# zkonduit/ezkl

Measured on AMD Instinct MI355X. Metric: BN254 G1 MSM pts/s (2^20 points per GPU; NTT 2^22 elems/s in extra), higher is better.
Workload: dtype u32x8 (254-bit modular integer, Montgomery)

## Files before the change

ezkl_amd/csrc/msm.hip:

```cpp
#include "common.hpp"
#include <deque>
#include <thread>
#include <chrono>
#include "curve.hpp"
#include "curve29.hpp"
#include "host64.hpp"
#include <string.h>

namespace ezkl {

static constexpr uint32_t MSM_MAX_PART_BITS = 12;
static constexpr uint32_t MSM_SPAN_HEAVY = 16;
static constexpr uint32_t MSM_PART_STAGE = 13312;
static constexpr uint32_t MSM_BINSORT_STAGE = 15360;
static constexpr uint32_t MSM_HEAVY_CHUNK = 256;
static constexpr uint32_t MSM_DIGIT_E = 8;
static constexpr uint32_t MSM_LMIN = 8;
static constexpr uint32_t MSM_MAX_BIG = 64;
static constexpr uint32_t MSM_BIG_BLOCKS = 64;
static constexpr uint32_t MSM_BIG_ROWS = 8;

__device__ __forceinline__ uint32_t msm_part_of(uint32_t bucket, uint32_t NP) { return bucket ? 1u + (bucket & (NP - 1u)) : 0u; }
__device__ __forceinline__ uint32_t msm_lane_len(const uint32_t* offsets, uint32_t nb, uint32_t nlanes, uint32_t lmin) {
    const uint32_t l = (uint32_t)(((uint64_t)offsets[nb] + nlanes - 1) / nlanes);
// ... 92 lines not shown
    double best_cost = 0;
    for (uint32_t W = 10; W <= 127; W++) {
        WinPlan p{W, 254 / W, 254 % W};
        if (p.cmax() > 23) continue;
        const double cost = (double)n * W + 4.0 * (double)((size_t)1 << (p.cmax() - 1));
        if (!best.W || cost < best_cost) { best = p; best_cost = cost; }
    }
    return best;
}

__global__ __launch_bounds__(256) void msm_precompute_kernel(const g1a_t* prev, g1a_t* next, size_t n, uint32_t c) {
    size_t i = (size_t)blockIdx.x * blockDim.x + threadIdx.x;
    if (i >= n) return;
    g1a_t p = ld_g1a(prev + i);
    g1x_t a = g1x_from_affine(p);
    for (uint32_t k = 0; k < c; k++) a = g1x_double(a);
    st_g1a(next + i, g1x_to_affine(a));
}

__global__ __launch_bounds__(256) void msm_table_to_r261_kernel(g1a_t* tab, size_t count) {
    size_t i = (size_t)blockIdx.x * blockDim.x + threadIdx.x;
    if (i >= count) return;
    fe_t k;
#pragma unroll
    for (int q = 0; q < 8; q++) k.v[q] = Fq29C::R261_32[q];
    g1a_t p = ld_g1a(tab + i);
    if (g1a_is_id(p)) return;
    p.x = Fq::mul(p.x, k);
    p.y = Fq::mul(p.y, k);
    st_g1a(tab + i, p);
}

__device__ __forceinline__ bool gt_half_r(const fe_t& s) {
    uint32_t d[8], c = 0, br = 0;
#pragma unroll
    for (int i = 0; i < 8; i++) d[i] = addc32(s.v[i], s.v[i], c);
#pragma unroll
    for (int i = 0; i < 8; i++) (void)subb32(d[i], FrP::MOD[i], br);
    return c != 0 || br == 0;
}
__device__ __forceinline__ fe_t msm_canon(const fe_t* scalars, size_t i, uint32_t& neg) {
    fe_t s = Fr::from_mont(ld_fe(scalars + i));
    neg = 0;
    if (gt_half_r(s)) {
        uint32_t br = 0;
#pragma unroll
        for (int k = 0; k < 8; k++) s.v[k] = subb32(FrP::MOD[k], s.v[k], br);
        neg = 1;
    }
    return s;
}
__device__ __forceinline__ uint32_t msm_take_bits(fe_t& s, uint32_t c) {
    const uint32_t d = s.v[0] & ((1u << c) - 1u);
#pragma unroll
    for (int k = 0; k < 7; k++) s.v[k] = __builtin_amdgcn_alignbit(s.v[k + 1], s.v[k], c);
    s.v[7] >>= c;
    return d;
}
template <class F>
__device__ __forceinline__ void msm_foreach_digit(fe_t s, uint32_t neg, const WinPlan& wp, F&& f) {
    uint32_t carry = 0;
    for (uint32_t w = 0; w < wp.W; w++) {
        const uint32_t c = wp.width(w), half = 1u << (c - 1);
        uint32_t raw = msm_take_bits(s, c) + carry;
        if (raw > half) {
            carry = 1;
            if (raw != (1u << c)) f(w, (1u << c) - raw - 1u, neg ^ 1u);
        } else {
            carry = 0;
            if (raw) f(w, raw - 1u, neg);
        }
    }
}

__device__ __forceinline__ bool msm_digit_step(fe_t& s, uint32_t neg, uint32_t c, uint32_t& carry, uint32_t& bucket, uint32_t& sign) {
    const uint32_t half = 1u << (c - 1);
    const uint32_t raw = msm_take_bits(s, c) + carry;
    if (raw > half) {
        carry = 1;
        bucket = (1u << c) - raw - 1u;
        sign = neg ^ 1u;
        return raw != (1u << c);
    }
    carry = 0;
    bucket = raw - 1u;
    sign = neg;
    return raw != 0;
}

__device__ __forceinline__ uint32_t msm_block_scan(uint32_t v, uint32_t* wsum, uint32_t& total) {
    const uint32_t lane = threadIdx.x & 63u, wave = threadIdx.x >> 6, nw = blockDim.x >> 6;
    uint32_t x = v;
#pragma unroll
    for (uint32_t d = 1; d < 64; d <<= 1) {
        const uint32_t y = __shfl_up(x, d, 64);
        if (lane >= d) x += y;
    }
    if (lane == 63) wsum[wave] = x;
    __syncthreads();
    if (wave == 0) {
        uint32_t s = lane < nw ? wsum[lane] : 0u;
#pragma unroll
        for (uint32_t d = 1; d < 16; d <<= 1) {
            const uint32_t y = __shfl_up(s, d, 64);
            if (lane >= d) s += y;
        }
        if (lane < nw) wsum[lane] = s;
    }
    __syncthreads();
    total = wsum[nw - 1];
    const uint32_t r = x + (wave ? wsum[wave - 1] : 0u);
    __syncthreads();
    return r;
}

__global__ __launch_bounds__(256) void msm_hist_kernel(const fe_t* scalars, size_t n, size_t per_block, WinPlan wp,
                                                       uint32_t LB, uint32_t NP, uint32_t* wg_hist, uint32_t* wg_cnt,
                                                       const fe_t* const* scal_list, uint32_t* zero_base, uint32_t zero_words, size_t bstride) {
    BOFF(); BSH(wg_hist); BSH(wg_cnt);
    if (scal_list) scalars = scal_list[blockIdx.z];
    if (zero_base) {
        BSH(zero_base);
        for (uint32_t i = blockIdx.x * 256 + threadIdx.x; i < zero_words; i += gridDim.x * 256) zero_base[i] = 0;
    }
    __shared__ uint32_t lh[(1u << MSM_MAX_PART_BITS) + 1];
    const uint32_t NQ = NP + 1;
    for (uint32_t p = threadIdx.x; p < NQ; p += 256) lh[p] = 0;
    __syncthreads();
    size_t lo = (size_t)blockIdx.x * per_block, hi = lo + per_block < n ? lo + per_block : n;
    for (size_t i0 = lo + threadIdx.x; i0 < hi; i0 += 4 * 256) {
        fe_t s[4];
        uint32_t neg[4], carry[4] = {0, 0, 0, 0};
#pragma unroll
        for (int q = 0; q < 4; q++) {
            const size_t i = i0 + (size_t)q * 256;
            if (i < hi) s[q] = msm_canon(scalars, i, neg[q]);
            else { s[q] = Fr::zero(); neg[q] = 0; }
        }
        for (uint32_t w = 0; w < wp.W; w++) {
            const uint32_t c = wp.width(w);
#pragma unroll
            for (int q = 0; q < 4; q++) {
                uint32_t bucket, sign;
                if (msm_digit_step(s[q], neg[q], c, carry[q], bucket, sign)) atomicAdd(&lh[msm_part_of(bucket, NP)], 1u);
            }
        }
    }
    __syncthreads();
    for (uint32_t p = threadIdx.x; p < NQ; p += 256) {
        wg_hist[(size_t)blockIdx.x * NQ + p] = lh[p];
        wg_cnt[(size_t)blockIdx.x * NQ + p] = lh[p];
    }
}
__global__ __launch_bounds__(1024) void msm_hist_scan_kernel(uint32_t* wg_hist, uint32_t G, uint32_t NP, uint32_t* part_count, size_t bstride) {
    BOFF(); BSH(wg_hist); BSH(part_count);
    __shared__ uint32_t sums[32][33];
    const uint32_t c = threadIdx.x & 31, j = threadIdx.x >> 5;
    const uint32_t p = blockIdx.x * 32 + c;
    const uint32_t chunk = (G + 31) / 32, g0 = j * chunk, g1 = g0 + chunk < G ? g0 + chunk : G;
    uint32_t s = 0;
    if (p < NP)
        for (uint32_t g = g0; g < g1; g++) s += wg_hist[(size_t)g * NP + p];
    sums[j][c] = s;
    __syncthreads();
    if (j == 0) {
        uint32_t run = 0;
        for (uint32_t q = 0; q < 32; q++) {
            uint32_t v = sums[q][c];
            sums[q][c] = run;
            run += v;
        }
        if (p < NP) part_count[p] = run;
    }
    __syncthreads();
    if (p < NP) {
        uint32_t run = sums[j][c];
        for (uint32_t g = g0; g < g1; g++) {
            uint32_t v = wg_hist[(size_t)g * NP + p];
            wg_hist[(size_t)g * NP + p] = run;
            run += v;
        }
    }
}
__device__ __forceinline__ void msm_part_scan_body(const uint32_t* part_count, uint32_t NQ, uint32_t* part_base, uint32_t* big_flag,
                                                   uint32_t* big_list, uint32_t* big_count, uint32_t* sh) {
    const uint32_t t = threadIdx.x;
    constexpr uint32_t PER = 5;
    uint32_t v[PER], sum = 0;
#pragma unroll
    for (uint32_t q = 0; q < PER; q++) {
        const uint32_t i = PER * t + q;
        v[q] = i < NQ ? part_count[i] : 0;
        sum += v[q];
    }
    uint32_t total;
    uint32_t run = msm_block_scan(sum, sh, total) - sum;
#pragma unroll
    for (uint32_t q = 0; q < PER; q++) {
        const uint32_t i = PER * t + q;
        if (i < NQ) part_base[i] = run;
        run += v[q];
    }
    if (t == 1023) part_base[NQ] = total;
#pragma unroll
    for (uint32_t q = 0; q < PER; q++) {
        const uint32_t i = PER * t + q;
        if (i == 0 || i >= NQ) continue;
        uint32_t slot = 0;
        if (v[q] > MSM_BINSORT_STAGE) {
            slot = atomicAdd(big_count, 1u);
            if (slot < MSM_MAX_BIG) big_list[slot] = i - 1;
            slot = slot < MSM_MAX_BIG ? slot + 1 : 0;
        }
        big_flag[i - 1] = slot;
    }
}
__global__ __launch_bounds__(1024) void msm_part_scan_kernel(const uint32_t* part_count, uint32_t NQ, uint32_t* part_base, uint32_t* big_flag,
                                                             uint32_t* big_list, uint32_t* big_count, size_t bstride) {
    BOFF(); BSH(part_count); BSH(part_base); BSH(big_flag); BSH(big_list); BSH(big_count);
    __shared__ uint32_t sh[1024];
    msm_part_scan_body(part_count, NQ, part_base, big_flag, big_list, big_count, sh);
}
__global__ __launch_bounds__(1024) void msm_partition_kernel(const fe_t* scalars, size_t n, size_t per_block, WinPlan wp,
                                                             uint32_t LB, uint32_t NP, size_t base_offset, size_t tab_stride,
                                                             const uint32_t* part_base, const uint32_t* wg_hist, const uint32_t* wg_cnt, uint2* entries,
                                                             uint32_t* vals, const fe_t* const* scal_list, size_t bstride) {
    BOFF(); BSH(part_base); BSH(wg_hist); BSH(wg_cnt); BSH(entries); BSH(vals);
    if (scal_list) scalars = scal_list[blockIdx.z];
    extern __shared__ uint32_t plds[];
    __shared__ uint32_t tsum[1024];
    const uint32_t NQ = NP + 1;
    uint32_t* start = plds;
    uint32_t* cursor = plds + (NQ + 1);
    uint32_t* gbase = plds + 2 * (NQ + 1);
    uint2* stage = reinterpret_cast<uint2*>(plds + 3 * (NQ + 1));
    const uint32_t t = threadIdx.x, T = blockDim.x;
    const uint32_t K = (NQ + T - 1) / T;
    uint32_t loc = 0;
    for (uint32_t q = 0; q < K; q++) {
        const uint32_t p = t * K + q;
        if (p < NQ) loc += wg_cnt[(size_t)blockIdx.x * NQ + p];
    }
    uint32_t total;
    uint32_t run = msm_block_scan(loc, tsum, total) - loc;
    for (uint32_t q = 0; q < K; q++) {
        const uint32_t p = t * K + q;
        if (p < NQ) {
            start[p] = run;
            cursor[p] = run;
            gbase[p] = part_base[p] + wg_hist[(size_t)blockIdx.x * NQ + p];
            run += wg_cnt[(size_t)blockIdx.x * NQ + p];
        }
    }
    __syncthreads();
    const size_t lo = (size_t)blockIdx.x * per_block, hi = lo + per_block < n ? lo + per_block : n;
    const size_t i = lo + t;
    if (i < hi) {
        uint32_t neg;
        fe_t s = msm_canon(scalars, i, neg);
        msm_foreach_digit(s, neg, wp, [&](uint32_t w, uint32_t bucket, uint32_t sign) {
            const uint32_t r = atomicAdd(&cursor[msm_part_of(bucket, NP)], 1u);
            stage[r] = make_uint2((uint32_t)(w * tab_stride + base_offset + i) | (sign << 31), bucket);
        });
    }
    __syncthreads();
    const uint32_t PB = 31 - __clz(NP);
    for (uint32_t idx = t; idx < total; idx += T) {
        const uint2 e = stage[idx];
        const uint32_t p = msm_part_of(e.y, NP);
        const uint32_t slot = gbase[p] + (idx - start[p]);
        if (p) entries[slot] = make_uint2(e.x, e.y >> PB);
        else vals[slot] = e.x;
    }
}
__device__ __forceinline__ uint32_t msm_wave_rank(uint32_t* cnt, uint32_t key) {
    const uint64_t active = __ballot(1);
    const uint32_t first = __builtin_amdgcn_readfirstlane(key);
    if (__ballot(key == first) == active) {
        const uint32_t rank = (uint32_t)__popcll(active & ((1ull << (threadIdx.x & 63u)) - 1ull));
        uint32_t base = 0;
        if (rank == 0) base = atomicAdd(&cnt[first], (uint32_t)__popcll(active));
        return (uint32_t)__builtin_amdgcn_readfirstlane(base) + rank;
    }
    return atomicAdd(&cnt[key], 1u);
}
__device__ __forceinline__ void msm_bins_scan(uint32_t* cnt, uint32_t* tsum, uint32_t nbins, uint32_t p, uint32_t beg, const uint32_t* part_base,
                                              bool emit, uint32_t* offsets, g1x29_t* buckets) {
    const uint32_t t = threadIdx.x;
    uint32_t loc[4], s = 0;
#pragma unroll
    for (int q = 0; q < 4; q++) {
        uint32_t j = t * 4 + q;
        loc[q] = j < nbins ? cnt[j] : 0;
        s += loc[q];
    }
    uint32_t total;
    uint32_t run = msm_block_scan(s, tsum, total) - s;
#pragma unroll
    for (int q = 0; q < 4; q++) {
        uint32_t j = t * 4 + q;
        if (j < nbins) {
            cnt[j] = run;
            if (emit) {
                const bool b0 = (p == 0 && j == 0);
                offsets[(size_t)p * nbins + j] = b0 ? part_base[0] : beg + run;
                if (b0 ? part_base[1] == part_base[0] : loc[q] == 0) st_f29(&buckets[(size_t)p * nbins + j].zz, Fq29::zero());
            }
        }
        run += loc[q];
    }
    __syncthreads();
}
__device__ __forceinline__ void msm_bigsort_count_body(const uint2* entries, const uint32_t* part_base, uint32_t LB, const uint32_t* big_list,
                                                       const uint32_t* big_count, uint32_t* bin_total, uint32_t* block_off, uint32_t* cnt, uint32_t bx,
                                                       uint32_t by, uint32_t rows);
__global__ __launch_bounds__(512) void msm_binsort_kernel(const uint2* entries, const uint32_t* part_base, uint32_t LB, uint32_t NP,
                                                          const uint32_t* big_flag, uint32_t* offsets, uint32_t* vals, g1x29_t* buckets,
                                                          const uint32_t* big_list, const uint32_t* big_count, uint32_t* bin_total, uint32_t* block_off,
                                                          size_t bstride) {
    BOFF(); BSH(entries); BSH(part_base); BSH(big_flag); BSH(offsets); BSH(vals); BSH(buckets);
    __shared__ uint32_t cnt[2048];
    __shared__ uint32_t tsum[512];
    extern __shared__ uint32_t stage[];
    if (blockIdx.x >= NP) {
        BSH(big_list); BSH(big_count); BSH(bin_total); BSH(block_off);
        const uint32_t w = blockIdx.x - NP;
        msm_bigsort_count_body(entries, part_base, LB, big_list, big_count, bin_total, block_off, cnt, w % MSM_BIG_BLOCKS, w / MSM_BIG_BLOCKS, MSM_BIG_ROWS);
        return;
// ... 97 lines not shown
                                                             uint32_t nb, uint32_t nlanes, g1x29_t* buckets, g1x29_t* head, g1x29_t* tail,
                                                             uint32_t* lane_first, uint32_t lmin, size_t bstride) {
    BOFF(); BSH(offsets); BSH(vals); BSH(buckets); BSH(head); BSH(tail); BSH(lane_first);
    const uint32_t t = blockIdx.x * blockDim.x + threadIdx.x;
    const uint32_t total = offsets[nb], L = msm_lane_len(offsets, nb, nlanes, lmin);
    const uint64_t k0w = (uint64_t)t * L;
    if (k0w >= total) return;
    const uint32_t k0 = (uint32_t)k0w;
    const uint32_t k1 = (uint64_t)k0 + L < total ? k0 + L : total;
    uint32_t lo = 0, hi = nb;
    while (hi - lo > 1) {
        uint32_t mid = (lo + hi) >> 1;
        if (offsets[mid] <= k0) lo = mid; else hi = mid;
    }
    uint32_t b = lo, bin_end = offsets[b + 1];
    uint32_t end_next = offsets[b + 2 <= nb ? b + 2 : nb];
    lane_first[t] = b;
    bool started_before = offsets[b] < k0;
    g1x29_t acc = g1x29_identity();
    MsmRec nxt = msm_fetch(tab, vals[k0]);
    uint32_t vn = k0 + 1 < k1 ? vals[k0 + 1] : 0u;
    for (uint32_t k = k0; k < k1; k++) {
        if (k == bin_end) {
            if (started_before) st_g1x29(head + t, acc); else st_g1x29(buckets + b, acc);
            acc.zz = Fq29::zero();
            started_before = false;
            b++;
            bin_end = end_next;
            if (bin_end == k) {
                uint32_t probes = 1;
                while (bin_end == k && probes < 4) { b++; bin_end = offsets[b + 1]; probes++; }
                if (bin_end == k) {
                    uint32_t lo2 = b + 1, hi2 = nb;
                    while (hi2 - lo2 > 1) {
                        uint32_t mid = (lo2 + hi2) >> 1;
                        if (offsets[mid] <= k) lo2 = mid; else hi2 = mid;
                    }
                    b = lo2;
                    bin_end = offsets[b + 1];
                }
            }
            end_next = offsets[b + 2 <= nb ? b + 2 : nb];
        }
        const MsmRec cur = nxt;
        nxt = msm_fetch(tab, vn);
        vn = k + 2 < k1 ? vals[k + 2] : 0u;
        acc = g1x29_add_mixed(acc, g1a29_unpack(cur.p), cur.neg);
    }
    if (k1 == bin_end) {
        if (started_before) st_g1x29(head + t, acc); else st_g1x29(buckets + b, acc);
    } else {
        if (started_before) st_g1x29(head + t, acc); else st_g1x29(tail + t, acc);
    }
}
EZ_D g1x29_t g1x29_shfl_down(const g1x29_t& p, uint32_t d) {
    g1x29_t r;
    const uint32_t* s = p.x.v;
    uint32_t* o = r.x.v;
#pragma unroll
    for (int k = 0; k < 36; k++) o[k] = __shfl_down(s[k], d);
    return r;
}
__global__ __launch_bounds__(256) void msm_fixup_boundary_tree_kernel(const uint32_t* offsets, uint32_t nb, uint32_t nlanes,
                                                                      const uint32_t* lane_first, const g1x29_t* head, const g1x29_t* tail, g1x29_t* buckets,
                                                                      uint32_t* heavy_list, uint32_t* heavy_count, uint32_t* chunk_list, uint32_t lmin,
                                                                      uint32_t span_heavy, size_t bstride) {
    BOFF(); BSH(offsets); BSH(lane_first); BSH(head); BSH(tail); BSH(buckets); BSH(heavy_list); BSH(heavy_count); BSH(chunk_list);
    const uint32_t t = blockIdx.x * blockDim.x + threadIdx.x + 1;
    const uint32_t lane = threadIdx.x & 63u;
    const uint32_t L = msm_lane_len(offsets, nb, nlanes, lmin);
    const uint64_t k0 = (uint64_t)t * L;
    bool cut = t < nlanes && k0 < offsets[nb];
    uint32_t b = 0, t1 = 0, t2 = 0;
    if (cut) {
        b = lane_first[t];
        const uint32_t beg = offsets[b], end = offsets[b + 1];
        cut = beg < k0;
        t1 = beg / L; t2 = (end - 1) / L;
    }
    if (cut && t2 - t1 > span_heavy) {
        if (t == t1 + 1 && t2 - t1 > MSM_HEAVY_CHUNK) heavy_list[atomicAdd(heavy_count, 1u)] = b;
        if ((t - t1 - 1) % MSM_HEAVY_CHUNK == 0) chunk_list[atomicAdd(heavy_count + 1, 1u)] = t;
        cut = false;
    }
    const uint32_t wave_last = t + (63u - lane);
    const uint32_t run = cut ? (t2 < wave_last ? t2 : wave_last) - t + 1u : 0u;
    uint32_t longest = run;
#pragma unroll
    for (uint32_t o = 32; o > 0; o >>= 1) {
        const uint32_t m = __shfl_xor(longest, o);
        longest = m > longest ? m : longest;
    }
    if (longest == 0) return;
    if (longest <= 2) {
        if (!cut || t != t1 + 1) return;
        g1x29_t acc = g1x29_add(ld_g1x29(tail + t1), ld_g1x29(head + t));
        for (uint32_t u = t + 1; u <= t2; u++) acc = g1x29_add(acc, ld_g1x29(head + u));
        st_g1x29(buckets + b, acc);
        return;
    }
    g1x29_t v = cut ? ld_g1x29(head + t) : g1x29_identity();
    uint32_t have = cut ? 1u : 0u;
#pragma unroll 1
    for (uint32_t d = 1; d < longest; d <<= 1) {
        const g1x29_t w = g1x29_shfl_down(v, d);
        const uint32_t hw = __shfl_down(have, d);
        if (have == d && run > d) {
            v = g1x29_add(v, w);
            have += hw;
        }
    }
    if (!cut || t != t1 + 1) return;
    g1x29_t acc = g1x29_add(ld_g1x29(tail + t1), v);
    for (uint32_t u = t + run; u <= t2; u++) acc = g1x29_add(acc, ld_g1x29(head + u));
    st_g1x29(buckets + b, acc);
}
__global__ __launch_bounds__(256) void msm_fixup_heavy1_kernel(const uint32_t* offsets, uint32_t nb, uint32_t nlanes, const uint32_t* lane_first, g1x29_t* head,
                                                               const g1x29_t* tail, g1x29_t* buckets, const uint32_t* chunk_list, const uint32_t* counts, uint32_t lmin,
                                                               uint32_t coop, size_t bstride) {
    BOFF(); BSH(offsets); BSH(lane_first); BSH(head); BSH(tail); BSH(buckets); BSH(chunk_list); BSH(counts);
    const uint32_t nchunks = counts[1], L = msm_lane_len(offsets, nb, nlanes, lmin);
    const uint32_t wave = threadIdx.x >> 6, lane = threadIdx.x & 63u;
    for (uint32_t ci = blockIdx.x * 4u + wave; ci < nchunks; ci += gridDim.x * 4u) {
        const uint32_t start = chunk_list[ci], b = lane_first[start];
        const uint32_t t2 = (offsets[b + 1] - 1) / L;
        const uint32_t stop = start + MSM_HEAVY_CHUNK - 1 < t2 ? start + MSM_HEAVY_CHUNK - 1 : t2;
        const uint32_t t1 = offsets[b] / L;
        const bool whole = t2 - t1 <= MSM_HEAVY_CHUNK;
        g1x29_t acc = (whole && lane == 63u) ? ld_g1x29(tail + t1) : g1x29_identity();
        for (uint32_t t = start + lane; t <= stop; t += 64) acc = g1x29_add(acc, ld_g1x29(head + t));
        acc = coop ? g1x29_group_sum_coop(acc, 64) : g1x29_group_sum(acc, 64);
        if (lane == 0) st_g1x29(whole ? buckets + b : head + start, acc);
    }
}
__global__ __launch_bounds__(256) void msm_fixup_heavy2_kernel(const uint32_t* offsets, uint32_t nb, uint32_t nlanes, const g1x29_t* head, const g1x29_t* tail,
                                                               const uint32_t* heavy_list, const uint32_t* counts, g1x29_t* buckets, uint32_t lmin, uint32_t coop, size_t bstride) {
    BOFF(); BSH(offsets); BSH(head); BSH(tail); BSH(heavy_list); BSH(counts); BSH(buckets);
    const uint32_t L = msm_lane_len(offsets, nb, nlanes, lmin);
    const uint32_t wave = threadIdx.x >> 6, lane = threadIdx.x & 63u;
    for (uint32_t h = blockIdx.x * 4u + wave; h < counts[0]; h += gridDim.x * 4u) {
        const uint32_t b = heavy_list[h];
        const uint32_t t1 = offsets[b] / L, t2 = (offsets[b + 1] - 1) / L;
        g1x29_t acc = lane == 63u ? ld_g1x29(tail + t1) : g1x29_identity();
        for (uint32_t t = t1 + 1 + lane * MSM_HEAVY_CHUNK; t <= t2; t += 64 * MSM_HEAVY_CHUNK) acc = g1x29_add(acc, ld_g1x29(head + t));
        acc = coop ? g1x29_group_sum_coop(acc, 64) : g1x29_group_sum(acc, 64);
        if (lane == 0) st_g1x29(buckets + b, acc);
    }
}

struct ReduceGeom {
    uint32_t wA, wB, wC;
    uint32_t wsA, wsB, wsC;
    uint32_t EA, GA, ET, GT;
};
__global__ __launch_bounds__(256, 2) void msm_reduce1_kernel(const g1x29_t* buckets, ReduceGeom g, g1x29_t* partA, g1x29_t* partT, size_t bstride) {
    BOFF(); BSH(buckets); BSH(partA); BSH(partT);
    const uint32_t idx = blockIdx.x * blockDim.x + threadIdx.x;
    g1x29_t acc = g1x29_identity();
    if (blockIdx.y == 0) {
        if (idx >= (g.GA << g.wA)) return;
        const uint32_t dA = idx & ((1u << g.wA) - 1u), grp = idx >> g.wA;
        for (uint32_t e = 0; e < g.EA; e++) acc = g1x29_add(acc, ld_g1x29(buckets + ((((size_t)grp * g.EA + e) << g.wA) | dA)));
        st_g1x29(partA + (size_t)dA * g.GA + grp, acc);
    } else {
        const uint32_t nT = 1u << (g.wB + g.wC);
        if (idx >= nT * g.GT) return;
        const uint32_t grp = idx % g.GT, t = idx / g.GT;
        for (uint32_t e = 0; e < g.ET; e++) acc = g1x29_add(acc, ld_g1x29(buckets + (((size_t)t << g.wA) | (e * g.GT + grp))));
        st_g1x29(partT + (size_t)t * g.GT + grp, acc);
    }
}
__global__ __launch_bounds__(64) void msm_reduce2_kernel(const g1x29_t* partA, const g1x29_t* partT, ReduceGeom g, g1x29_t* SA, g1x29_t* T, uint32_t lanesA,
                                                         uint32_t lanesT, uint32_t blocksA, uint32_t coop, size_t bstride) {
    BOFF(); BSH(partA); BSH(partT); BSH(SA); BSH(T);
    const bool isA = blockIdx.x < blocksA;
    const uint32_t lanes = isA ? lanesA : lanesT, per = 64 / lanes;
    const uint32_t o = (isA ? blockIdx.x : blockIdx.x - blocksA) * per + threadIdx.x / lanes, j = threadIdx.x % lanes;
    const uint32_t nout = isA ? (1u << g.wA) : (1u << (g.wB + g.wC)), G = isA ? g.GA : g.GT;
    g1x29_t acc = g1x29_identity();
    if (o < nout) {
        const g1x29_t* src = (isA ? partA : partT) + (size_t)o * G;
        for (uint32_t i = j; i < G; i += lanes) acc = g1x29_add(acc, ld_g1x29(src + i));
    }
    acc = (coop && lanes >= 4) ? g1x29_group_sum_coop(acc, lanes) : g1x29_group_sum(acc, lanes);
    if (j == 0 && o < nout) st_g1x29((isA ? SA : T) + o, acc);
}
__global__ __launch_bounds__(256) void msm_planes_kernel(const g1x29_t* SA, const g1x29_t* T, ReduceGeom g, g1x29_t* planes, g1x29_t* planes_host, uint32_t coop,
                                                         size_t bstride) {
    BOFF(); BSH(SA); BSH(T); BSH(planes);
    __shared__ uint4 sh[9 * 4];
    uint32_t id = blockIdx.x, field = 0, j = 0;
    if (id > 0) {
        id -= 1;
        if (id < g.wA) { field = 1; j = id; }
        else if (id < g.wA + g.wB) { field = 2; j = id - g.wA; }
        else { field = 3; j = id - g.wA - g.wB; }
    }
    const uint32_t nA = 1u << g.wA, nT = 1u << (g.wB + g.wC);
    g1x29_t acc = g1x29_identity();
    auto with_bit = [](uint32_t k, uint32_t bit) { return ((k >> bit) << (bit + 1)) | (1u << bit) | (k & ((1u << bit) - 1u)); };
    if (field == 0) {
        for (uint32_t d = threadIdx.x; d < nA; d += 256) acc = g1x29_add(acc, ld_g1x29(SA + d));
    } else if (field == 1) {
        for (uint32_t k = threadIdx.x; k < nA / 2; k += 256) acc = g1x29_add(acc, ld_g1x29(SA + with_bit(k, j)));
    } else {
        const uint32_t sh_bits = field == 2 ? j : g.wB + j;
        for (uint32_t k = threadIdx.x; k < nT / 2; k += 256) acc = g1x29_add(acc, ld_g1x29(T + with_bit(k, sh_bits)));
    }
    acc = (coop & 8u) ? g1x29_block256_sum_coop_full(acc, sh) : coop ? g1x29_block256_sum_coop(acc, sh) : g1x29_block256_sum(acc, sh);
    if (threadIdx.x == 0) {
        const uint32_t ws = field == 1 ? g.wsA : field == 2 ? g.wsB : g.wsC;
        const uint32_t slot = field == 0 ? 0u : 1u + ws + j;
        st_g1x29(planes + slot, acc);
        if (planes_host) st_g1x29(planes_host + (size_t)blockIdx.z * 32 + slot, acc);
    }
}

static int table_build(Ctx* c, hipStream_t st, const Bases* b, bool wait) {
    MsmTable t;
    t.n = b->n;
    t.wp = pick_plan(b->n);
    if ((size_t)t.wp.W * t.n >= ((size_t)1 << 31)) return EZKL_ERR_UNSUPPORTED;
    EZ_HIP(hipMalloc(&t.tab, (size_t)t.wp.W * t.n * sizeof(g1a_t)));
    EZ_HIP(hipMemcpyAsync(t.tab, b->pts, t.n * sizeof(g1a_t), hipMemcpyDeviceToDevice, st));
    for (uint32_t w = 1; w < t.wp.W; w++)
        hipLaunchKernelGGL(msm_precompute_kernel, dim3(cdiv(t.n, 256)), dim3(256), 0, st, t.tab + (size_t)(w - 1) * t.n,
                           t.tab + (size_t)w * t.n, t.n, t.wp.width(w - 1));
    hipLaunchKernelGGL(msm_table_to_r261_kernel, dim3(cdiv((size_t)t.wp.W * t.n, 256)), dim3(256), 0, st, t.tab, (size_t)t.wp.W * t.n);
    EZ_HIP(hipGetLastError());
    EZ_HIP(hipEventCreateWithFlags(&t.ready, hipEventDisableTiming));
    EZ_HIP(hipEventRecord(t.ready, st));
    if (wait) {
        EZ_HIP(hipStreamSynchronize(st));
        t.synced = true;
    }
    g_tables[b] = t;
    return EZKL_OK;
}
static int table_get(Ctx* c, hipStream_t st, const Bases* b, MsmTable** out) {
    auto it = g_tables.find(b);
    if (it == g_tables.end()) {
        int rc = table_build(c, st, b, true);
        if (rc) return rc;
        it = g_tables.find(b);
    }
    if (!it->second.synced) {
        EZ_HIP(hipEventSynchronize(it->second.ready));
        it->second.synced = true;
    }
    *out = &it->second;
    return EZKL_OK;
}
int msm_table_prepare(Ctx* c, const Bases* b) {
    if (g_tables.count(b)) return EZKL_OK;
    if (!g_table_stream) EZ_HIP(hipStreamCreateWithFlags(&g_table_stream, hipStreamNonBlocking));
    return table_build(c, g_table_stream, b, false);
}
void msm_table_drop(const Bases* b) {
    auto it = g_tables.find(b);
    if (it != g_tables.end()) {
        if (it->second.ready) { (void)hipEventSynchronize(it->second.ready); (void)hipEventDestroy(it->second.ready); }
        (void)hipFree(it->second.tab);
        g_tables.erase(it);
    }
}

static constexpr size_t MSM_MAX_GROUP = 16;
static int slot_prepare(MsmSlot& sl, size_t bytes, size_t msms = 1) {
    if (!sl.st) {
        EZ_HIP(stream_create_prio(&sl.st, "EZKL_HIP_PRIO_MSM", 0));
        EZ_HIP(hipEventCreateWithFlags(&sl.done, hipEventDisableTiming));
        EZ_HIP(hipHostMalloc((void**)&sl.list_pinned, MSM_MAX_GROUP * sizeof(void*), hipHostMallocDefault));
    }
    if (msms > sl.pinned_msms) {
        if (sl.pinned) {
            EZ_HIP(hipStreamSynchronize(sl.st));
            EZ_HIP(hipHostFree(sl.pinned));
            sl.pinned = nullptr;
        }
        EZ_HIP(hipHostMalloc((void**)&sl.pinned, msms * 32 * sizeof(g1x29_t), hipHostMallocDefault));
        EZ_HIP(hipHostGetDevicePointer(&sl.pinned_dev, sl.pinned, 0));
        sl.pinned_msms = msms;
    }
    if (bytes > sl.scratch_bytes) {
        if (sl.scratch) {
            EZ_HIP(hipStreamSynchronize(sl.st));
            EZ_HIP(hipFree(sl.scratch));
            sl.scratch = nullptr;
            sl.scratch_bytes = 0;
        }
        size_t want = bytes + (bytes >> 4);
        EZ_HIP(hipMalloc((void**)&sl.scratch, want));
        sl.scratch_bytes = want;
    }
    return EZKL_OK;
}
static int msm_finish(MsmSlot& sl, void* out_host = nullptr, bool release = true) {
    if (!out_host) out_host = sl.out;
    EZ_HIP(hipEventSynchronize(sl.done));
    for (uint32_t j = 0; j < sl.count; j++) {
        const uint32_t* hp = sl.pinned + (size_t)j * 32 * 36;
        h64::xyzz acc = h64::identity();
        for (int k = (int)sl.bits - 1; k >= 0; k--) {
            acc = h64::dbl(acc);
            acc = h64::add(acc, h64::from_limbs29_point(hp + 36 * (1 + k)));
        }
        acc = h64::add(acc, h64::from_limbs29_point(hp));
        h64::aff r = h64::to_affine(acc);
        memcpy((uint8_t*)out_host + 64 * (size_t)j, &r, 64);
    }
    if (release) sl.busy = false;
    return EZKL_OK;
}

static size_t msm_group_size(const MsmTable* T, size_t n, bool small_scalars, size_t batch = 0) {
    if (const char* e = getenv("EZKL_MSM_GROUP")) {
        const int v = atoi(e);
        if (v >= 1 && v <= (int)MSM_MAX_GROUP) return (size_t)v;
    }
    (void)T; (void)n; (void)batch;
    if (small_scalars) {
        static const int small = [] { const char* e = getenv("EZKL_MSM_GROUP_SMALL"); const int v = e ? atoi(e) : 0; return v >= 1 && v <= (int)MSM_MAX_GROUP ? v : 6; }();
        return (size_t)small;
    }
    static const int big = [] { const char* e = getenv("EZKL_MSM_GROUP_BIG"); const int v = e ? atoi(e) : 0; return v >= 1 && v <= (int)MSM_MAX_GROUP ? v : 4; }();
    return (size_t)big;
}
static int msm_enqueue(Ctx* c, MsmSlot& sl, hipStream_t st, MsmTable* T, size_t base_offset, const fe_t* const* cols, size_t count, size_t n, bool timed) {
    int rc = EZKL_OK;
    if (count < 1 || count > MSM_MAX_GROUP) return EZKL_ERR_INVALID;
    const unsigned Z = (unsigned)count;
    const fe_t* scalars = cols[0];
    const WinPlan wp = T->wp;
    const uint32_t W = wp.W, bits = wp.cmax() - 1;
    const uint32_t nb = 1u << bits;
    const size_t npairs = n * W;
    uint32_t PB = bits < 10 ? bits : 10;
    while (PB < bits && PB < MSM_MAX_PART_BITS && (npairs >> PB) > (size_t)MSM_BINSORT_STAGE * 9 / 10) PB++;
    const uint32_t LB = bits - PB, NP = 1u << PB;
    int& acc_blocks_per_cu = msm_state().acc_blocks_per_cu;
    if (!acc_blocks_per_cu) {
        EZ_HIP(hipFuncSetAttribute((const void*)msm_binsort_kernel, hipFuncAttributeMaxDynamicSharedMemorySize, 96 * 1024));
        EZ_HIP(hipFuncSetAttribute((const void*)msm_partition_kernel, hipFuncAttributeMaxDynamicSharedMemorySize, 144 * 1024));
        EZ_HIP(hipOccupancyMaxActiveBlocksPerMultiprocessor(&acc_blocks_per_cu, msm_accumulate_kernel, 256, 0));
        if (acc_blocks_per_cu < 1) acc_blocks_per_cu = 1;
    }
    const size_t resident = (size_t)acc_blocks_per_cu * 256 * c->num_cus;
    const size_t load = npairs >> bits, per_lane = load * 9 / 10 > 40 ? load * 9 / 10 : 40;
    size_t rounds = npairs / (resident * per_lane);
    if (rounds < 1) rounds = 1;
    uint32_t L = (uint32_t)((npairs + resident * rounds - 1) / (resident * rounds));
    if (L < 8) L = 8;
    if (const char* e = getenv("EZKL_MSM_L")) {
        const int v = atoi(e);
        if (v > 0 && v < (1 << 20)) L = (uint32_t)v;
    }
    const uint32_t nlanes = cdiv(npairs, L);
    static const uint32_t lmin = [] { const char* e = getenv("EZKL_MSM_LMIN"); const int v = e ? atoi(e) : 0; return (uint32_t)(v >= 1 && v <= 4096 ? v : (int)MSM_LMIN); }();
    constexpr uint32_t coop = 7;
    static const uint32_t span_heavy = [] { const char* e = getenv("EZKL_MSM_SPAN"); const int v = e ? atoi(e) : 0; return (uint32_t)(v >= 1 && v <= 4096 ? v : (int)MSM_SPAN_HEAVY); }();
    ReduceGeom rg;
    memset(&rg, 0, sizeof rg);
    if (LB > 0) {
        rg.wA = LB; rg.wsA = PB;
        rg.wB = (PB + 1) / 2; rg.wsB = 0;
        rg.wC = PB - rg.wB; rg.wsC = rg.wB;
    } else {
        rg.wA = (bits + 2) / 3; rg.wsA = 0;
        rg.wB = (bits - rg.wA + 1) / 2; rg.wsB = rg.wA;
        rg.wC = bits - rg.wA - rg.wB; rg.wsC = rg.wA + rg.wB;
    }
    {
        const uint32_t rows = 1u << (rg.wB + rg.wC), cols = 1u << rg.wA;
        uint32_t E = MSM_DIGIT_E;
        if (const char* e = getenv("EZKL_MSM_E")) {
            const int v = atoi(e);
            if (v > 0 && v <= 1024 && (v & (v - 1)) == 0) E = (uint32_t)v;
        }
        rg.EA = rows < E ? rows : E; rg.GA = rows / rg.EA;
        rg.ET = cols < E ? cols : E; rg.GT = cols / rg.ET;
    }
    const uint32_t nA = 1u << rg.wA, nT = 1u << (rg.wB + rg.wC);
    const uint32_t n_partA = nA * rg.GA, n_partT = nT * rg.GT;
    const uint32_t nplanes = 1 + bits;
    size_t per_block = MSM_PART_STAGE / W / 64 * 64;
    {
        const size_t lds_words = (144u << 10) / 4, fixed = 3 * ((size_t)NP + 2);
        const size_t fit = lds_words > fixed ? (lds_words - fixed) / (2 * (size_t)W) / 64 * 64 : 64;
        if (per_block > fit) per_block = fit;
    }
    if (per_block > 1024) per_block = 1024;
    if (per_block < 64) per_block = 64;
    const unsigned sgrid = cdiv(n, per_block);
    auto al = [](size_t x) { return (x + 255) & ~(size_t)255; };
    size_t off = 0;
    auto carve = [&](size_t bytes) { size_t o = off; off += al(bytes); return o; };
    size_t o_list = carve(MSM_MAX_GROUP * sizeof(void*));
    size_t o_ent = carve(npairs * 8), o_vals = carve(npairs * 4), o_offs = carve(((size_t)nb + 1) * 4);
    const uint32_t NQ = NP + 1;
    size_t o_pcnt = carve((NQ + 1) * 4), o_pbase = carve((NQ + 1) * 4), o_wgh = carve((size_t)sgrid * NQ * 4), o_wgc = carve((size_t)sgrid * NQ * 4);
    size_t o_heavy = carve((size_t)nb * 4), o_chunks = carve(((size_t)nlanes + 1) * 4);
    const size_t nbins = (size_t)1 << LB;
    size_t o_hcnt = carve(256), o_btot = carve(MSM_MAX_BIG * nbins * 4), o_planes = carve((size_t)nplanes * sizeof(g1x29_t));
    const size_t zero_bytes = off - o_hcnt;
    size_t o_bflag = carve((size_t)NP * 4), o_blist = carve(MSM_MAX_BIG * 4),
           o_boff = carve((size_t)MSM_MAX_BIG * MSM_BIG_BLOCKS * nbins * 4);
    size_t o_lfirst = carve((size_t)nlanes * 4);
    size_t o_bkt = carve((size_t)nb * sizeof(g1x29_t));
    size_t o_head = carve((size_t)nlanes * sizeof(g1x29_t)), o_tail = carve((size_t)nlanes * sizeof(g1x29_t));
    size_t o_partA = carve((size_t)n_partA * sizeof(g1x29_t)), o_partT = carve((size_t)n_partT * sizeof(g1x29_t));
    size_t o_SA = carve((size_t)nA * sizeof(g1x29_t)), o_T = carve((size_t)nT * sizeof(g1x29_t));
    const size_t bstride = count > 1 ? off : 0;
    rc = slot_prepare(sl, off * count, count);
    if (rc) return rc;
    uint8_t* S = sl.scratch;
    const fe_t* const* scal_list = nullptr;
    if (count > 1) {
        for (size_t j = 0; j < count; j++) sl.list_pinned[j] = cols[j];
        EZ_HIP(hipMemcpyAsync(S + o_list, sl.list_pinned, count * sizeof(void*), hipMemcpyHostToDevice, st));
        scal_list = (const fe_t* const*)(S + o_list);
    }
    uint2* entries = (uint2*)(S + o_ent);
    uint32_t* vals = (uint32_t*)(S + o_vals);
    uint32_t* offs = (uint32_t*)(S + o_offs);
    uint32_t *pcnt = (uint32_t*)(S + o_pcnt), *pbase = (uint32_t*)(S + o_pbase), *wghist = (uint32_t*)(S + o_wgh), *wgcnt = (uint32_t*)(S + o_wgc);
    uint32_t *heavy = (uint32_t*)(S + o_heavy), *hcnt = (uint32_t*)(S + o_hcnt), *chunks = (uint32_t*)(S + o_chunks);
    uint32_t* lfirst = (uint32_t*)(S + o_lfirst);
    uint32_t *bflag = (uint32_t*)(S + o_bflag), *blist = (uint32_t*)(S + o_blist), *btot = (uint32_t*)(S + o_btot), *boff = (uint32_t*)(S + o_boff);
    uint32_t* bcnt = hcnt + 2;
    g1x29_t *bkt = (g1x29_t*)(S + o_bkt), *head = (g1x29_t*)(S + o_head), *tail = (g1x29_t*)(S + o_tail);
    g1x29_t *partA = (g1x29_t*)(S + o_partA), *partT = (g1x29_t*)(S + o_partT), *SA = (g1x29_t*)(S + o_SA), *TT = (g1x29_t*)(S + o_T);
    g1x29_t* planes = (g1x29_t*)(S + o_planes);

    hipEvent_t m0 = nullptr, m1 = nullptr, a0 = nullptr, a1 = nullptr;
    bool timed_chain = timed;
    if (timed) {
        const char* tm = getenv("EZKL_HIP_TIMING");
        if (tm && !strcmp(tm, "none")) timed = timed_chain = false;
        else if (tm && !strcmp(tm, "kernel")) timed_chain = false;
    }
    if (timed) {
        if (timed_chain && (rc = ev_pair(c, "msm", &m0, &m1))) return rc;
        if ((rc = ev_pair(c, "msm_accumulate", &a0, &a1))) return rc;
        if (timed_chain) EZ_HIP(hipEventRecord(m0, st));
    }
    hipLaunchKernelGGL(msm_hist_kernel, dim3(sgrid, 1, Z), dim3(256), 0, st, scalars, n, per_block, wp, LB, NP, wghist, wgcnt, scal_list, hcnt,
                       (uint32_t)(zero_bytes / 4), bstride);
    hipLaunchKernelGGL(msm_hist_scan_kernel, dim3(cdiv(NQ, 32), 1, Z), dim3(1024), 0, st, wghist, sgrid, NQ, pcnt, bstride);
    hipLaunchKernelGGL(msm_part_scan_kernel, dim3(1, 1, Z), dim3(1024), 0, st, pcnt, NQ, pbase, bflag, blist, bcnt, bstride);
    hipLaunchKernelGGL(msm_partition_kernel, dim3(sgrid, 1, Z), dim3((unsigned)per_block), (3 * ((size_t)NQ + 1) + 2 * per_block * W) * 4, st, scalars, n, per_block, wp,
                       LB, NP, base_offset, T->n, pbase, wghist, wgcnt, entries, vals, scal_list, bstride);
    hipLaunchKernelGGL(msm_binsort_kernel, dim3(NP + MSM_BIG_BLOCKS * MSM_BIG_ROWS, 1, Z), dim3(512), MSM_BINSORT_STAGE * 4, st, entries, pbase, LB, NP, bflag, offs,
                       vals, bkt, blist, bcnt, btot, boff, bstride);
    hipLaunchKernelGGL(msm_bigsort_scatter_kernel, dim3(MSM_BIG_BLOCKS, MSM_BIG_ROWS, Z), dim3(512), 0, st, entries, pbase, LB, blist, bcnt, btot, boff, offs,
                       vals, bkt, bstride);
    if (timed) EZ_HIP(hipEventRecord(a0, st));
    hipLaunchKernelGGL(msm_accumulate_kernel, dim3(cdiv(nlanes, 256), 1, Z), dim3(256), 0, st, T->tab, offs, vals, nb, nlanes, bkt, head, tail,
                       lfirst, lmin, bstride);
    if (timed) EZ_HIP(hipEventRecord(a1, st));
    if (nlanes > 1)
    {
        hipLaunchKernelGGL(msm_fixup_boundary_tree_kernel, dim3(cdiv(nlanes - 1, 256), 1, Z), dim3(256), 0, st, offs, nb, nlanes, lfirst, head, tail, bkt,
                           heavy, hcnt, chunks, lmin, span_heavy, bstride);
    }
    {
        size_t max_heavy = nlanes / span_heavy + 1;
        const size_t heavy_wgs = (max_heavy + 3) / 4;
        unsigned hb = (unsigned)(heavy_wgs < (size_t)c->num_cus * 4 ? heavy_wgs : (size_t)c->num_cus * 4);
        size_t max_chunks = nlanes / MSM_HEAVY_CHUNK + max_heavy;
        const size_t chunk_wgs = (max_chunks + 3) / 4;
        unsigned cb = (unsigned)(chunk_wgs < (size_t)c->num_cus * 4 ? chunk_wgs : (size_t)c->num_cus * 4);
        hipLaunchKernelGGL(msm_fixup_heavy1_kernel, dim3(cb, 1, Z), dim3(256), 0, st, offs, nb, nlanes, lfirst, head, tail, bkt, chunks, hcnt, lmin, coop & 4u, bstride);
        hipLaunchKernelGGL(msm_fixup_heavy2_kernel, dim3(hb, 1, Z), dim3(256), 0, st, offs, nb, nlanes, head, tail, heavy, hcnt, bkt, lmin, coop & 4u, bstride);
    }
    {
        const uint32_t th = n_partA > n_partT ? n_partA : n_partT;
        hipLaunchKernelGGL(msm_reduce1_kernel, dim3(cdiv(th, 256), 2, Z), dim3(256), 0, st, bkt, rg, partA, partT, bstride);
        auto pow2_le = [](uint32_t x) { uint32_t p = 1; while (p * 2 <= x) p *= 2; return p; };
        uint32_t lanesA = pow2_le(rg.GA < 64 ? rg.GA : 64), lanesT = pow2_le(rg.GT < 64 ? rg.GT : 64);
        auto waves = [&](uint32_t nout, uint32_t lanes) { return cdiv(nout, 64 / lanes); };
        while (waves(nA, lanesA) + waves(nT, lanesT) > (unsigned)c->num_cus * 4 && (lanesA > 1 || lanesT > 1)) {
            if (lanesT > 1 && waves(nT, lanesT) >= waves(nA, lanesA)) lanesT >>= 1; else if (lanesA > 1) lanesA >>= 1; else lanesT >>= 1;
        }
        const uint32_t blocksA = waves(nA, lanesA);
        hipLaunchKernelGGL(msm_reduce2_kernel, dim3(blocksA + waves(nT, lanesT), 1, Z), dim3(64), 0, st, partA, partT, rg, SA, TT, lanesA, lanesT, blocksA, coop & 1u, bstride);
        hipLaunchKernelGGL(msm_planes_kernel, dim3(nplanes, 1, Z), dim3(256), 0, st, SA, TT, rg, planes, (g1x29_t*)sl.pinned_dev,
                           coop & 10u, bstride);
    }
    EZ_HIP(hipGetLastError());
    if (getenv("EZKL_MSM_DEBUG")) {
        uint32_t hc = 0;
        EZ_HIP(hipMemcpyAsync(&hc, hcnt, 4, hipMemcpyDeviceToHost, st));
        EZ_HIP(hipStreamSynchronize(st));
        fprintf(stderr, "[msm] n=%zu W=%u bits=%u L=%u nlanes=%u heavy=%u\n", n, W, bits, L, nlanes, hc);
    }
    if (timed_chain) EZ_HIP(hipEventRecord(m1, st));
    EZ_HIP(hipEventRecord(sl.done, st));
    sl.bits = bits;
    sl.count = (uint32_t)count;
    sl.busy = true;
    return EZKL_OK;
}
static int msm_run_groups(Ctx* c, MsmTable* T, size_t base_offset, const fe_t* const* cols, size_t batch, size_t n, void* out_host,
                          const hipEvent_t* wait_ev, bool small_scalars) {
    const size_t G = msm_group_size(T, n, small_scalars, batch);
    static const bool dbg = getenv("EZKL_MSM_DEBUG") != nullptr;
    if (dbg) fprintf(stderr, "[ezkl_hip] msm batch: %zu columns of %zu points, %s scalars, groups of %zu\n", batch, n, small_scalars ? "witness-shaped" : "general", G);
    int rc = EZKL_OK;
    size_t gi = 0;
    for (size_t j0 = 0; j0 < batch && !rc; gi++) {
        size_t cnt = batch - j0 < G ? batch - j0 : G;
        if (wait_ev && j0 > 0) {
            const size_t left = batch - j0;
            cnt = left <= 2 ? 1 : std::min(G, (left + 1) / 2);
        }
        MsmSlot& sl = g_slots[gi % MSM_SLOTS];
        if (sl.busy) rc = msm_finish(sl);
        if (!rc) rc = slot_prepare(sl, 0);
        for (size_t j = 0; wait_ev && j < cnt && !rc; j++)
            if (hipStreamWaitEvent(sl.st, wait_ev[j0 + j], 0) != hipSuccess) rc = EZKL_ERR_HIP;
        if (!rc) {
            sl.out = (uint8_t*)out_host + 64 * j0;
            rc = msm_enqueue(c, sl, sl.st, T, base_offset, cols + j0, cnt, n, false);
        }
        j0 += cnt;
    }
    for (size_t k = 0; k < (size_t)MSM_SLOTS; k++) {
        MsmSlot& sl = g_slots[(gi + k) % MSM_SLOTS];
        if (!sl.busy) continue;
        if (!rc) rc = msm_finish(sl);
        else { (void)hipStreamSynchronize(sl.st); sl.busy = false; }
    }
    return rc;
}

struct MsmBatch;
static MsmBatch* g_open_batch_fwd();
int msm_run(Ctx* c, hipStream_t st, const Bases* b, size_t base_offset, const fe_t* scalars, size_t n, void* out_host) {
    if (g_open_batch_fwd()) return EZKL_ERR_INVALID;
    if (n == 0) { memset(out_host, 0, 64); return EZKL_OK; }
    MsmTable* T = nullptr;
    int rc = table_get(c, st, b, &T);
    if (rc) return rc;
    MsmSlot& sl = g_slots[0];
    if (sl.busy) return EZKL_ERR_INVALID;
    static const bool host_timing = getenv("EZKL_MSM_HOST_TIMING") != nullptr;
    if (!host_timing) {
        if ((rc = msm_enqueue(c, sl, st, T, base_offset, &scalars, 1, n, true))) return rc;
        return msm_finish(sl, out_host);
    }
    auto now = [] { return std::chrono::duration<double, std::micro>(std::chrono::steady_clock::now().time_since_epoch()).count(); };
    static double acc[3] = {0, 0, 0};
    static int calls = 0;
    const double t0 = now();
    if ((rc = msm_enqueue(c, sl, st, T, base_offset, &scalars, 1, n, true))) return rc;
    const double t1 = now();
    EZ_HIP(hipEventSynchronize(sl.done));
    const double t2 = now();
    rc = msm_finish(sl, out_host);
    const double t3 = now();
    acc[0] += t1 - t0; acc[1] += t2 - t1; acc[2] += t3 - t2;
    if (++calls % 50 == 0) {
        fprintf(stderr, "[msm host] n=%zu per call: enqueue %.1f us, wait for the GPU %.1f us, host tail %.1f us\n", n, acc[0] / 50, acc[1] / 50, acc[2] / 50);
        acc[0] = acc[1] = acc[2] = 0;
    }
    return rc;
}

int msm_call_start(Ctx* c, std::unique_lock<std::recursive_mutex>& lk, const Bases* b, size_t base_offset, const fe_t* scalars, size_t n, int* slot_out) {
    if (g_open_batch_fwd() || n == 0) return EZKL_ERR_INVALID;
    MsmTable* T = nullptr;
    int rc = table_get(c, c->stream, b, &T);
    if (rc) return rc;
    int k = -1;
    for (;;) {
        for (int i = 0; i < MSM_CALL_SLOTS && k < 0; i++)
            if (!g_call_claimed[i]) k = i;
        if (k >= 0) break;
        bool all_mine = true;
        for (int i = 0; i < MSM_CALL_SLOTS; i++) all_mine = all_mine && g_call_owner[i] == std::this_thread::get_id();
        if (all_mine) return EZKL_ERR_BUSY;
        lk.unlock();
        std::this_thread::yield();
        lk.lock();
    }
    MsmSlot& sl = g_call_slots[k];
    g_call_claimed[k] = true;
    g_call_finishing[k] = false;
    g_call_owner[k] = std::this_thread::get_id();
    rc = slot_prepare(sl, 0);
    if (!rc) {
        hipError_t e = hipSuccess;
        const hipError_t q = hipStreamQuery(c->stream);
        if (q != hipSuccess) {
            (void)hipGetLastError();
            if (!g_call_order_ev) e = hipEventCreateWithFlags(&g_call_order_ev, hipEventDisableTiming);
            if (e == hipSuccess) e = hipEventRecord(g_call_order_ev, c->stream);
            if (e == hipSuccess) e = hipStreamWaitEvent(sl.st, g_call_order_ev, 0);
        }
        if (e != hipSuccess) rc = set_hip_error(e, "msm_call_start", __FILE__, __LINE__);
    }
    if (!rc) rc = msm_enqueue(c, sl, sl.st, T, base_offset, &scalars, 1, n, true);
    if (rc) { g_call_claimed[k] = false; g_call_owner[k] = std::thread::id(); return rc; }
    *slot_out = k;
    return EZKL_OK;
}
int msm_call_finish(Ctx* c, std::unique_lock<std::recursive_mutex>& lk, int k, void* out_host) {
    (void)c;
    if (k < 0 || k >= MSM_CALL_SLOTS || !g_call_claimed[k] || g_call_finishing[k] || !g_call_slots[k].busy) return EZKL_ERR_INVALID;
    MsmSlot& sl = g_call_slots[k];
    g_call_finishing[k] = true;
    lk.unlock();
    const int rc = msm_finish(sl, out_host, false);
    lk.lock();
    sl.busy = false;
    g_call_finishing[k] = false;
    g_call_claimed[k] = false;
    g_call_owner[k] = std::thread::id();
    return rc;
}
int msm_run_concurrent(Ctx* c, std::unique_lock<std::recursive_mutex>& lk, const Bases* b, size_t base_offset, const fe_t* scalars, size_t n, void* out_host) {
    if (g_open_batch_fwd()) return EZKL_ERR_INVALID;
    if (n == 0) { memset(out_host, 0, 64); return EZKL_OK; }
    int k = -1;
    static const bool host_timing = getenv("EZKL_MSM_HOST_TIMING") != nullptr;
    auto now = [] { return std::chrono::duration<double, std::micro>(std::chrono::steady_clock::now().time_since_epoch()).count(); };
    const double t0 = host_timing ? now() : 0;
    int rc = msm_call_start(c, lk, b, base_offset, scalars, n, &k);
    if (rc) return rc;
    if (!host_timing) return msm_call_finish(c, lk, k, out_host);
    static double acc[3] = {0, 0, 0};
    static int calls = 0;
    const double t1 = now();
    (void)hipEventSynchronize(g_call_slots[k].done);
    const double t2 = now();
    rc = msm_call_finish(c, lk, k, out_host);
    const double t3 = now();
    acc[0] += t1 - t0; acc[1] += t2 - t1; acc[2] += t3 - t2;
// ... 357 lines not shown
```

Before: 784.9 million.

## Fuse MSM bucket reduce stages and keep histogram scan values in registers

Merges the two-stage bucket reduction into one kernel. Each 256-thread block now accumulates its groups, sums them within each wave and then across waves through shared memory, writing partial sums per output. This removes the partA/partT intermediate buffers and one kernel launch, and the planes kernel now sums the extra PA/PT partials. Separately, the histogram scan caches up to 32 per-thread values in registers so the second pass does not re-read global memory. The cost is more register pressure and a changed partition geometry that the planes kernel must index correctly.

```diff
diff --git a/ezkl_amd/csrc/msm.hip b/ezkl_amd/csrc/msm.hip
--- a/ezkl_amd/csrc/msm.hip
+++ b/ezkl_amd/csrc/msm.hip
@@ -268,15 +268,27 @@
         wg_cnt[(size_t)blockIdx.x * NQ + p] = lh[p];
     }
 }
+static constexpr uint32_t MSM_SCAN_KEEP = 32;
 __global__ __launch_bounds__(1024) void msm_hist_scan_kernel(uint32_t* wg_hist, uint32_t G, uint32_t NP, uint32_t* part_count, size_t bstride) {
     BOFF(); BSH(wg_hist); BSH(part_count);
     __shared__ uint32_t sums[32][33];
     const uint32_t c = threadIdx.x & 31, j = threadIdx.x >> 5;
     const uint32_t p = blockIdx.x * 32 + c;
     const uint32_t chunk = (G + 31) / 32, g0 = j * chunk, g1 = g0 + chunk < G ? g0 + chunk : G;
+    const bool keep = chunk <= MSM_SCAN_KEEP;
+    uint32_t kv[MSM_SCAN_KEEP];
     uint32_t s = 0;
-    if (p < NP)
+    if (keep) {
+#pragma unroll
+        for (uint32_t q = 0; q < MSM_SCAN_KEEP; q++) {
+            const uint32_t g = g0 + q;
+            kv[q] = p < NP && g < g1 ? wg_hist[(size_t)g * NP + p] : 0u;
+        }
+#pragma unroll
+        for (uint32_t q = 0; q < MSM_SCAN_KEEP; q++) s += kv[q];
+    } else if (p < NP) {
         for (uint32_t g = g0; g < g1; g++) s += wg_hist[(size_t)g * NP + p];
+    }
     sums[j][c] = s;
     __syncthreads();
     if (j == 0) {
@@ -289,7 +301,15 @@
         if (p < NP) part_count[p] = run;
     }
     __syncthreads();
-    if (p < NP) {
+    if (keep) {
+        uint32_t run = sums[j][c];
+#pragma unroll
+        for (uint32_t q = 0; q < MSM_SCAN_KEEP; q++) {
+            const uint32_t g = g0 + q;
+            if (p < NP && g < g1) wg_hist[(size_t)g * NP + p] = run;
+            run += kv[q];
+        }
+    } else if (p < NP) {
         uint32_t run = sums[j][c];
         for (uint32_t g = g0; g < g1; g++) {
             uint32_t v = wg_hist[(size_t)g * NP + p];
@@ -693,38 +713,59 @@
     uint32_t wA, wB, wC;
     uint32_t wsA, wsB, wsC;
     uint32_t EA, GA, ET, GT;
+    uint32_t PA, PT;
 };
-__global__ __launch_bounds__(256, 2) void msm_reduce1_kernel(const g1x29_t* buckets, ReduceGeom g, g1x29_t* partA, g1x29_t* partT, size_t bstride) {
-    BOFF(); BSH(buckets); BSH(partA); BSH(partT);
-    const uint32_t idx = blockIdx.x * blockDim.x + threadIdx.x;
+__global__ __launch_bounds__(256, 2) void msm_reduce1_kernel(const g1x29_t* buckets, ReduceGeom g, g1x29_t* SA, g1x29_t* T, uint32_t coop, size_t bstride) {
+    BOFF(); BSH(buckets); BSH(SA); BSH(T);
+    __shared__ uint4 sh[9 * 4];
+    const bool isA = blockIdx.y == 0;
+    const uint32_t G = isA ? g.GA : g.GT, R = G < 256 ? G : 256, P = isA ? g.PA : g.PT;
+    const uint32_t nout = isA ? (1u << g.wA) : (1u << (g.wB + g.wC));
+    const uint32_t limit = nout * G;
+    if (blockIdx.x * 256u >= limit) return;
+    const uint32_t idx = blockIdx.x * 256u + threadIdx.x;
+    const uint32_t part = idx / R, j = idx % R;
+    const uint32_t o = part / P, grp = (part % P) * R + j;
     g1x29_t acc = g1x29_identity();
-    if (blockIdx.y == 0) {
-        if (idx >= (g.GA << g.wA)) return;
-        const uint32_t dA = idx & ((1u << g.wA) - 1u), grp = idx >> g.wA;
-        for (uint32_t e = 0; e < g.EA; e++) acc = g1x29_add(acc, ld_g1x29(buckets + ((((size_t)grp * g.EA + e) << g.wA) | dA)));
-        st_g1x29(partA + (size_t)dA * g.GA + grp, acc);
-    } else {
-        const uint32_t nT = 1u << (g.wB + g.wC);
-        if (idx >= nT * g.GT) return;
-        const uint32_t grp = idx % g.GT, t = idx / g.GT;
-        for (uint32_t e = 0; e < g.ET; e++) acc = g1x29_add(acc, ld_g1x29(buckets + (((size_t)t << g.wA) | (e * g.GT + grp))));
-        st_g1x29(partT + (size_t)t * g.GT + grp, acc);
-    }
-}
-__global__ __launch_bounds__(64) void msm_reduce2_kernel(const g1x29_t* partA, const g1x29_t* partT, ReduceGeom g, g1x29_t* SA, g1x29_t* T, uint32_t lanesA,
-                                                         uint32_t lanesT, uint32_t blocksA, uint32_t coop, size_t bstride) {
-    BOFF(); BSH(partA); BSH(partT); BSH(SA); BSH(T);
-    const bool isA = blockIdx.x < blocksA;
-    const uint32_t lanes = isA ? lanesA : lanesT, per = 64 / lanes;
-    const uint32_t o = (isA ? blockIdx.x : blockIdx.x - blocksA) * per + threadIdx.x / lanes, j = threadIdx.x % lanes;
-    const uint32_t nout = isA ? (1u << g.wA) : (1u << (g.wB + g.wC)), G = isA ? g.GA : g.GT;
-    g1x29_t acc = g1x29_identity();
-    if (o < nout) {
-        const g1x29_t* src = (isA ? partA : partT) + (size_t)o * G;
-        for (uint32_t i = j; i < G; i += lanes) acc = g1x29_add(acc, ld_g1x29(src + i));
-    }
-    acc = (coop && lanes >= 4) ? g1x29_group_sum_coop(acc, lanes) : g1x29_group_sum(acc, lanes);
-    if (j == 0 && o < nout) st_g1x29((isA ? SA : T) + o, acc);
+    if (idx < limit) {
+        if (isA) {
+            for (uint32_t e = 0; e < g.EA; e++) acc = g1x29_add(acc, ld_g1x29(buckets + ((((size_t)grp * g.EA + e) << g.wA) | o)));
+        } else {
+            for (uint32_t e = 0; e < g.ET; e++) acc = g1x29_add(acc, ld_g1x29(buckets + (((size_t)o << g.wA) | (e * g.GT + grp))));
+        }
+    }
+    const uint32_t ww = R < 64 ? R : 64;
+    acc = (coop && ww >= 4) ? g1x29_group_sum_coop(acc, ww) : g1x29_group_sum(acc, ww);
+    if (R > 64) {
+        const uint32_t wave = threadIdx.x >> 6, nw = R >> 6, first = wave & ~(nw - 1u);
+        if ((threadIdx.x & 63u) == 0) {
+            const uint32_t* s = acc.x.v;
+#pragma unroll
+            for (int k = 0; k < 9; k++) sh[k * 4 + wave] = make_uint4(s[4 * k], s[4 * k + 1], s[4 * k + 2], s[4 * k + 3]);
+        }
+        __syncthreads();
+        auto wave_total = [&](uint32_t v) {
+            g1x29_t r;
+            uint32_t* d = r.x.v;
+#pragma unroll
+            for (int k = 0; k < 9; k++) {
+                const uint4 t = sh[k * 4 + first + v];
+                d[4 * k] = t.x; d[4 * k + 1] = t.y; d[4 * k + 2] = t.z; d[4 * k + 3] = t.w;
+            }
+            return r;
+        };
+        acc = wave_total(0);
+#pragma unroll 1
+        for (uint32_t v = 1; v < nw; v++) {
+            const g1x29_t b = wave_total(v);
+            bool special = true;
+            g1x29_t r = acc;
+            if (coop) r = g1x29_add_quad(acc, b, special);
+            if (special) r = g1x29_add(acc, b);
+            acc = r;
+        }
+    }
+    if (j == 0 && idx < limit) st_g1x29((isA ? SA : T) + part, acc);
 }
 __global__ __launch_bounds__(256) void msm_planes_kernel(const g1x29_t* SA, const g1x29_t* T, ReduceGeom g, g1x29_t* planes, g1x29_t* planes_host, uint32_t coop,
                                                          size_t bstride) {
@@ -740,13 +781,14 @@
     const uint32_t nA = 1u << g.wA, nT = 1u << (g.wB + g.wC);
     g1x29_t acc = g1x29_identity();
     auto with_bit = [](uint32_t k, uint32_t bit) { return ((k >> bit) << (bit + 1)) | (1u << bit) | (k & ((1u << bit) - 1u)); };
+    const uint32_t lpA = 31u - (uint32_t)__clz(g.PA), lpT = 31u - (uint32_t)__clz(g.PT);
     if (field == 0) {
-        for (uint32_t d = threadIdx.x; d < nA; d += 256) acc = g1x29_add(acc, ld_g1x29(SA + d));
+        for (uint32_t d = threadIdx.x; d < nA * g.PA; d += 256) acc = g1x29_add(acc, ld_g1x29(SA + d));
     } else if (field == 1) {
-        for (uint32_t k = threadIdx.x; k < nA / 2; k += 256) acc = g1x29_add(acc, ld_g1x29(SA + with_bit(k, j)));
+        for (uint32_t k = threadIdx.x; k < nA / 2 * g.PA; k += 256) acc = g1x29_add(acc, ld_g1x29(SA + with_bit(k, j + lpA)));
     } else {
         const uint32_t sh_bits = field == 2 ? j : g.wB + j;
-        for (uint32_t k = threadIdx.x; k < nT / 2; k += 256) acc = g1x29_add(acc, ld_g1x29(T + with_bit(k, sh_bits)));
+        for (uint32_t k = threadIdx.x; k < nT / 2 * g.PT; k += 256) acc = g1x29_add(acc, ld_g1x29(T + with_bit(k, sh_bits + lpT)));
     }
     acc = (coop & 8u) ? g1x29_block256_sum_coop_full(acc, sh) : coop ? g1x29_block256_sum_coop(acc, sh) : g1x29_block256_sum(acc, sh);
     if (threadIdx.x == 0) {
@@ -920,6 +962,7 @@
         }
         rg.EA = rows < E ? rows : E; rg.GA = rows / rg.EA;
         rg.ET = cols < E ? cols : E; rg.GT = cols / rg.ET;
+        rg.PA = rg.GA > 256 ? rg.GA / 256 : 1; rg.PT = rg.GT > 256 ? rg.GT / 256 : 1;
     }
     const uint32_t nA = 1u << rg.wA, nT = 1u << (rg.wB + rg.wC);
     const uint32_t n_partA = nA * rg.GA, n_partT = nT * rg.GT;
@@ -949,8 +992,7 @@
     size_t o_lfirst = carve((size_t)nlanes * 4);
     size_t o_bkt = carve((size_t)nb * sizeof(g1x29_t));
     size_t o_head = carve((size_t)nlanes * sizeof(g1x29_t)), o_tail = carve((size_t)nlanes * sizeof(g1x29_t));
-    size_t o_partA = carve((size_t)n_partA * sizeof(g1x29_t)), o_partT = carve((size_t)n_partT * sizeof(g1x29_t));
-    size_t o_SA = carve((size_t)nA * sizeof(g1x29_t)), o_T = carve((size_t)nT * sizeof(g1x29_t));
+    size_t o_SA = carve((size_t)nA * rg.PA * sizeof(g1x29_t)), o_T = carve((size_t)nT * rg.PT * sizeof(g1x29_t));
     const size_t bstride = count > 1 ? off : 0;
     rc = slot_prepare(sl, off * count, count);
     if (rc) return rc;
@@ -970,7 +1012,7 @@
     uint32_t *bflag = (uint32_t*)(S + o_bflag), *blist = (uint32_t*)(S + o_blist), *btot = (uint32_t*)(S + o_btot), *boff = (uint32_t*)(S + o_boff);
     uint32_t* bcnt = hcnt + 2;
     g1x29_t *bkt = (g1x29_t*)(S + o_bkt), *head = (g1x29_t*)(S + o_head), *tail = (g1x29_t*)(S + o_tail);
-    g1x29_t *partA = (g1x29_t*)(S + o_partA), *partT = (g1x29_t*)(S + o_partT), *SA = (g1x29_t*)(S + o_SA), *TT = (g1x29_t*)(S + o_T);
+    g1x29_t *SA = (g1x29_t*)(S + o_SA), *TT = (g1x29_t*)(S + o_T);
     g1x29_t* planes = (g1x29_t*)(S + o_planes);
 
     hipEvent_t m0 = nullptr, m1 = nullptr, a0 = nullptr, a1 = nullptr;
@@ -1016,15 +1058,7 @@
     }
     {
         const uint32_t th = n_partA > n_partT ? n_partA : n_partT;
-        hipLaunchKernelGGL(msm_reduce1_kernel, dim3(cdiv(th, 256), 2, Z), dim3(256), 0, st, bkt, rg, partA, partT, bstride);
-        auto pow2_le = [](uint32_t x) { uint32_t p = 1; while (p * 2 <= x) p *= 2; return p; };
-        uint32_t lanesA = pow2_le(rg.GA < 64 ? rg.GA : 64), lanesT = pow2_le(rg.GT < 64 ? rg.GT : 64);
-        auto waves = [&](uint32_t nout, uint32_t lanes) { return cdiv(nout, 64 / lanes); };
-        while (waves(nA, lanesA) + waves(nT, lanesT) > (unsigned)c->num_cus * 4 && (lanesA > 1 || lanesT > 1)) {
-            if (lanesT > 1 && waves(nT, lanesT) >= waves(nA, lanesA)) lanesT >>= 1; else if (lanesA > 1) lanesA >>= 1; else lanesT >>= 1;
-        }
-        const uint32_t blocksA = waves(nA, lanesA);
-        hipLaunchKernelGGL(msm_reduce2_kernel, dim3(blocksA + waves(nT, lanesT), 1, Z), dim3(64), 0, st, partA, partT, rg, SA, TT, lanesA, lanesT, blocksA, coop & 1u, bstride);
+        hipLaunchKernelGGL(msm_reduce1_kernel, dim3(cdiv(th, 256), 2, Z), dim3(256), 0, st, bkt, rg, SA, TT, coop & 1u, bstride);
         hipLaunchKernelGGL(msm_planes_kernel, dim3(nplanes, 1, Z), dim3(256), 0, st, SA, TT, rg, planes, (g1x29_t*)sl.pinned_dev,
                            coop & 10u, bstride);
     }
```

Result: no change. 789.0 million, median of 6 (+0.5%).
